# sampotter/butterfly

Measured on AMD Instinct MI355X. Metric: butterfly matvecs/sec (2D Helmholtz HODBF apply), higher is better.
Workload: dtype c128

## Files before the change

butterfly_amd/csrc/bfhip_stage_mfma.h:

```cpp
#ifndef BFHIP_STAGE_MFMA_H
#define BFHIP_STAGE_MFMA_H

#define BF_MF_TABCAP 1792u
#define BF_MF_TABPAD 24u
#define BF_MF_SPAN_BYTES (1u << 31)
#ifndef BF_MFMA_WAVES_PER_SIMD
#define BF_MFMA_WAVES_PER_SIMD 2
#endif
#ifndef BF_MF_XCD_RUN
#define BF_MF_XCD_RUN 32u
#endif
#ifndef BF_MF_WG_WAVES
#define BF_MF_WG_WAVES 1u
#endif
#ifndef BF_MFMA_MIN_RHS
#define BF_MFMA_MIN_RHS 2
#endif
#ifndef BF_MF_QUARTER
#define BF_MF_QUARTER 1
#endif

typedef double bf_d4 __attribute__((ext_vector_type(4)));
typedef int bf_i4 __attribute__((ext_vector_type(4)));
union BfFrag { bf_u4 u; double d[2]; };

__device__ __forceinline__ bf_i4 bfMakeRsrc(void const *base, uint32_t bytes) {
  uint64_t const b = (uint64_t)base;
  bf_i4 r;
  r.x = __builtin_amdgcn_readfirstlane((int)(uint32_t)b);
  r.y = __builtin_amdgcn_readfirstlane((int)((uint32_t)(b >> 32) & 0xffffu));
  r.z = __builtin_amdgcn_readfirstlane((int)bytes);
  r.w = 0x00020000;
  return r;
}
#ifndef BF_MF_A_POLICY
#define BF_MF_A_POLICY "nt"
#endif
template <int STREAM, int OFF> __device__ __forceinline__ void bfFragLoad(BfFrag &f, uint32_t voff, bf_i4 rsrc, uint32_t soff) {
  if (STREAM) asm volatile("buffer_load_dwordx4 %0, %1, %2, %3 offen offset:%4 " BF_MF_A_POLICY : "=v"(f.u) : "v"(voff), "s"(rsrc), "s"(soff), "n"(OFF));
  else asm volatile("buffer_load_dwordx4 %0, %1, %2, %3 offen offset:%4" : "=v"(f.u) : "v"(voff), "s"(rsrc), "s"(soff), "n"(OFF));
}
template <int N> __device__ __forceinline__ void bfFragWait(BfFrag &f) { asm volatile("s_waitcnt vmcnt(%1)" : "+v"(f.u) : "n"(N)); }
template <int N> __device__ __forceinline__ void bfFragWait(BfFrag &f, BfFrag &g) { asm volatile("s_waitcnt vmcnt(%2)" : "+v"(f.u), "+v"(g.u) : "n"(N)); }

struct BfMfSeg {
  bf_i4 ra, rx;
  uint32_t voffA;
  uint32_t cX;
  uint32_t stepA;
  uint32_t ksteps;
};

__device__ __forceinline__ void bfMfmaExact(bf_d4 &re, bf_d4 &im, BfFrag const &a, BfFrag const &x) {
  re = __builtin_amdgcn_mfma_f64_16x16x4f64(a.d[0], x.d[0], re, 0, 0, 0);
  re = __builtin_amdgcn_mfma_f64_16x16x4f64(a.d[1], x.d[1], re, 0, 0, 1);
  im = __builtin_amdgcn_mfma_f64_16x16x4f64(a.d[0], x.d[1], im, 0, 0, 0);
  im = __builtin_amdgcn_mfma_f64_16x16x4f64(a.d[1], x.d[0], im, 0, 0, 0);
}
template <int MS, int SET>
__device__ __forceinline__ void bfMfmaRequestA(BfFrag (&a)[2][2], BfMfSeg const &sg, uint32_t soffA) {
  bfFragLoad<1, 0>(a[SET][0], sg.voffA, sg.ra, soffA);
  if (MS > 1) bfFragLoad<1, 256>(a[SET][1], sg.voffA, sg.ra, soffA);
}
template <int T>
__device__ __forceinline__ void bfMfmaRequestX(BfFrag (&x)[4], BfMfSeg const &sg, uint32_t voffX) {
  bfFragLoad<0, 256 * T>(x[T], voffX, sg.rx, 0);
}
template <int NT, int MS, int SET, int T, bool GAUSS>
__device__ __forceinline__ void bfMfmaTile(bf_d4 (&acc)[3][2][4], BfFrag (&a)[2][2], BfFrag (&x)[4], double (&as)[2], BfMfSeg const &sg, uint32_t voffXnext) {
  if (T < NT) {
    constexpr int TT = T < NT ? T : 0;
    constexpr int pending = NT - 1 + MS;
    if (T == 0 && MS > 1) asm volatile("s_waitcnt vmcnt(%3)" : "+v"(a[SET][0].u), "+v"(a[SET][1].u), "+v"(x[0].u) : "n"(pending));
    else if (T == 0) asm volatile("s_waitcnt vmcnt(%2)" : "+v"(a[SET][0].u), "+v"(x[0].u) : "n"(pending));
    else asm volatile("s_waitcnt vmcnt(%1)" : "+v"(x[TT].u) : "n"(pending));
    if (GAUSS) {
      if (T == 0) {
        as[0] = a[SET][0].d[0] + a[SET][0].d[1];
        if (MS > 1) as[1] = a[SET][1].d[0] + a[SET][1].d[1];
      }
      double const xs = x[TT].d[0] + x[TT].d[1];
#pragma unroll
      for (int m = 0; m < MS; ++m) {
        acc[0][m][TT] = __builtin_amdgcn_mfma_f64_16x16x4f64(a[SET][m].d[0], x[TT].d[0], acc[0][m][TT], 0, 0, 0);
        acc[1][m][TT] = __builtin_amdgcn_mfma_f64_16x16x4f64(a[SET][m].d[1], x[TT].d[1], acc[1][m][TT], 0, 0, 0);
        acc[2][m][TT] = __builtin_amdgcn_mfma_f64_16x16x4f64(as[m], xs, acc[2][m][TT], 0, 0, 0);
      }
    } else {
#pragma unroll
      for (int m = 0; m < MS; ++m) bfMfmaExact(acc[0][m][TT], acc[1][m][TT], a[SET][m], x[TT]);
    }
    __builtin_amdgcn_sched_barrier(0);
    bfMfmaRequestX<TT>(x, sg, voffXnext);
    __builtin_amdgcn_sched_barrier(0);
  }
}
template <int NT, int MS, bool GAUSS = true>
__device__ __forceinline__ void bfMfmaSegment(bf_d4 (&acc)[3][2][4], BfMfSeg const &sg, uint32_t const *tab, uint32_t lk) {
  BfFrag a[2][2], x[4];
  double as[2];
  uint32_t ti = lk;
  uint32_t soffA = 0;
  {
    uint32_t const v0 = tab[ti] + sg.cX;
    bfMfmaRequestA<MS, 0>(a, sg, soffA);
    bfMfmaRequestX<0>(x, sg, v0);
    if (NT > 1) bfMfmaRequestX<1>(x, sg, v0);
    if (NT > 2) bfMfmaRequestX<2>(x, sg, v0);
    if (NT > 3) bfMfmaRequestX<3>(x, sg, v0);
  }
  uint32_t t1 = tab[ti + 4], t2 = tab[ti + 8];
  ti += 12;
  for (uint32_t ks = 0; ks < sg.ksteps; ks += 2) {
    uint32_t const v1 = t1 + sg.cX, v2 = t2 + sg.cX;
    t1 = tab[ti];
    t2 = tab[ti + 4];
    ti += 8;
    soffA += sg.stepA;
    __builtin_amdgcn_sched_barrier(0);
    bfMfmaRequestA<MS, 1>(a, sg, soffA);
    __builtin_amdgcn_sched_barrier(0);
    bfMfmaTile<NT, MS, 0, 0, GAUSS>(acc, a, x, as, sg, v1);
    bfMfmaTile<NT, MS, 0, 1, GAUSS>(acc, a, x, as, sg, v1);
    bfMfmaTile<NT, MS, 0, 2, GAUSS>(acc, a, x, as, sg, v1);
    bfMfmaTile<NT, MS, 0, 3, GAUSS>(acc, a, x, as, sg, v1);
    soffA += sg.stepA;
    bfMfmaRequestA<MS, 0>(a, sg, soffA);
    __builtin_amdgcn_sched_barrier(0);
    bfMfmaTile<NT, MS, 1, 0, GAUSS>(acc, a, x, as, sg, v2);
    bfMfmaTile<NT, MS, 1, 1, GAUSS>(acc, a, x, as, sg, v2);
    bfMfmaTile<NT, MS, 1, 2, GAUSS>(acc, a, x, as, sg, v2);
    bfMfmaTile<NT, MS, 1, 3, GAUSS>(acc, a, x, as, sg, v2);
  }
  asm volatile("s_waitcnt vmcnt(0)" : "+v"(a[0][0].u), "+v"(a[0][MS > 1 ? 1 : 0].u), "+v"(x[0].u), "+v"(x[NT > 1 ? 1 : 0].u), "+v"(x[NT > 2 ? 2 : 0].u), "+v"(x[NT > 3 ? 3 : 0].u));
}

template <int MS, int QT, int SET>
__device__ __forceinline__ void bfMfmaRequestAQ(BfFrag (&a)[2], BfFrag (&aq)[2][3], BfMfSeg const &sg, uint32_t voffAq, uint32_t soffA) {
  if (MS > 0) bfFragLoad<1, 0>(a[SET], sg.voffA, sg.ra, soffA);
  bfFragLoad<1, 256 * MS>(aq[SET][0], voffAq, sg.ra, soffA);
  if (QT > 1) bfFragLoad<1, 256 * MS + 64>(aq[SET][1], voffAq, sg.ra, soffA);
  if (QT > 2) bfFragLoad<1, 256 * MS + 128>(aq[SET][2], voffAq, sg.ra, soffA);
}
template <int MS, int QT, int SET, int T>
__device__ __forceinline__ void bfMfmaTileQ(bf_d4 (&acc)[3][4], double (&accq)[3][3][4], BfFrag (&a)[2], BfFrag (&aq)[2][3], BfFrag (&x)[4], double &as, double (&asq)[3],
                                            BfMfSeg const &sg, uint32_t voffXnext) {
  constexpr int pending = 4 - 1 + MS + QT;
  if (T == 0) {
    if (MS > 0 && QT == 1) asm volatile("s_waitcnt vmcnt(%3)" : "+v"(a[SET].u), "+v"(aq[SET][0].u), "+v"(x[0].u) : "n"(pending));
    else if (MS > 0 && QT == 2) asm volatile("s_waitcnt vmcnt(%4)" : "+v"(a[SET].u), "+v"(aq[SET][0].u), "+v"(aq[SET][1].u), "+v"(x[0].u) : "n"(pending));
    else if (MS > 0) asm volatile("s_waitcnt vmcnt(%5)" : "+v"(a[SET].u), "+v"(aq[SET][0].u), "+v"(aq[SET][1].u), "+v"(aq[SET][2].u), "+v"(x[0].u) : "n"(pending));
    else if (QT == 1) asm volatile("s_waitcnt vmcnt(%2)" : "+v"(aq[SET][0].u), "+v"(x[0].u) : "n"(pending));
    else if (QT == 2) asm volatile("s_waitcnt vmcnt(%3)" : "+v"(aq[SET][0].u), "+v"(aq[SET][1].u), "+v"(x[0].u) : "n"(pending));
    else asm volatile("s_waitcnt vmcnt(%4)" : "+v"(aq[SET][0].u), "+v"(aq[SET][1].u), "+v"(aq[SET][2].u), "+v"(x[0].u) : "n"(pending));
    if (MS > 0) as = a[SET].d[0] + a[SET].d[1];
#pragma unroll
    for (int q = 0; q < QT; ++q) asq[q] = aq[SET][q].d[0] + aq[SET][q].d[1];
  } else asm volatile("s_waitcnt vmcnt(%1)" : "+v"(x[T].u) : "n"(pending));
  double const xs = x[T].d[0] + x[T].d[1];
  if (MS > 0) {
    acc[0][T] = __builtin_amdgcn_mfma_f64_16x16x4f64(a[SET].d[0], x[T].d[0], acc[0][T], 0, 0, 0);
    acc[1][T] = __builtin_amdgcn_mfma_f64_16x16x4f64(a[SET].d[1], x[T].d[1], acc[1][T], 0, 0, 0);
    acc[2][T] = __builtin_amdgcn_mfma_f64_16x16x4f64(as, xs, acc[2][T], 0, 0, 0);
  }
#pragma unroll
  for (int q = 0; q < QT; ++q) {
    accq[0][q][T] = __builtin_amdgcn_mfma_f64_4x4x4f64(aq[SET][q].d[0], x[T].d[0], accq[0][q][T], 0, 0, 0);
    accq[1][q][T] = __builtin_amdgcn_mfma_f64_4x4x4f64(aq[SET][q].d[1], x[T].d[1], accq[1][q][T], 0, 0, 0);
    accq[2][q][T] = __builtin_amdgcn_mfma_f64_4x4x4f64(asq[q], xs, accq[2][q][T], 0, 0, 0);
  }
  __builtin_amdgcn_sched_barrier(0);
  bfMfmaRequestX<T>(x, sg, voffXnext);
  __builtin_amdgcn_sched_barrier(0);
}
template <int MS, int QT>
__device__ __forceinline__ void bfMfmaSegmentQ(bf_d4 (&acc)[3][4], double (&accq)[3][3][4], BfMfSeg const &sg, uint32_t voffAq, uint32_t const *tab, uint32_t lk) {
  BfFrag a[2], aq[2][3], x[4];
  double as = 0, asq[3];
  uint32_t ti = lk;
  uint32_t soffA = 0;
  {
    uint32_t const v0 = tab[ti] + sg.cX;
    bfMfmaRequestAQ<MS, QT, 0>(a, aq, sg, voffAq, soffA);
    bfMfmaRequestX<0>(x, sg, v0);
    bfMfmaRequestX<1>(x, sg, v0);
    bfMfmaRequestX<2>(x, sg, v0);
    bfMfmaRequestX<3>(x, sg, v0);
  }
  uint32_t t1 = tab[ti + 4], t2 = tab[ti + 8];
  ti += 12;
  for (uint32_t ks = 0; ks < sg.ksteps; ks += 2) {
    uint32_t const v1 = t1 + sg.cX, v2 = t2 + sg.cX;
    t1 = tab[ti];
    t2 = tab[ti + 4];
    ti += 8;
    soffA += sg.stepA;
    __builtin_amdgcn_sched_barrier(0);
    bfMfmaRequestAQ<MS, QT, 1>(a, aq, sg, voffAq, soffA);
    __builtin_amdgcn_sched_barrier(0);
    bfMfmaTileQ<MS, QT, 0, 0>(acc, accq, a, aq, x, as, asq, sg, v1);
    bfMfmaTileQ<MS, QT, 0, 1>(acc, accq, a, aq, x, as, asq, sg, v1);
    bfMfmaTileQ<MS, QT, 0, 2>(acc, accq, a, aq, x, as, asq, sg, v1);
    bfMfmaTileQ<MS, QT, 0, 3>(acc, accq, a, aq, x, as, asq, sg, v1);
    soffA += sg.stepA;
    bfMfmaRequestAQ<MS, QT, 0>(a, aq, sg, voffAq, soffA);
    __builtin_amdgcn_sched_barrier(0);
    bfMfmaTileQ<MS, QT, 1, 0>(acc, accq, a, aq, x, as, asq, sg, v2);
    bfMfmaTileQ<MS, QT, 1, 1>(acc, accq, a, aq, x, as, asq, sg, v2);
    bfMfmaTileQ<MS, QT, 1, 2>(acc, accq, a, aq, x, as, asq, sg, v2);
    bfMfmaTileQ<MS, QT, 1, 3>(acc, accq, a, aq, x, as, asq, sg, v2);
  }
  if (MS > 0) asm volatile("s_waitcnt vmcnt(0)" : "+v"(a[0].u) :: "memory");
  if (QT == 1) asm volatile("s_waitcnt vmcnt(0)" : "+v"(aq[0][0].u), "+v"(x[0].u), "+v"(x[1].u), "+v"(x[2].u), "+v"(x[3].u));
  else if (QT == 2) asm volatile("s_waitcnt vmcnt(0)" : "+v"(aq[0][0].u), "+v"(aq[0][1].u), "+v"(x[0].u), "+v"(x[1].u), "+v"(x[2].u), "+v"(x[3].u));
  else asm volatile("s_waitcnt vmcnt(0)" : "+v"(aq[0][0].u), "+v"(aq[0][1].u), "+v"(aq[0][2].u), "+v"(x[0].u), "+v"(x[1].u), "+v"(x[2].u), "+v"(x[3].u));
}
template <int MS, int QT>
__device__ __forceinline__ void bfMfmaStoreQ(StageParams const &p, BfDevItem const &it, uint32_t mr, uint32_t s0, uint32_t q0, double (&accq)[3][3][4], bool hasIdentity, int lane) {
  uint32_t const nrhs = p.nrhs, np = it.numPieces;
  double2 *out = (it.mrFlags & BF_ITEM_OUT_Y) ? (double2 *)p.y : (double2 *)p.temp;
  uint32_t const qmax = nrhs - 1 - q0;
  uint32_t lane2 = (uint32_t)lane;
  asm volatile("" : "+v"(lane2));
  uint32_t const li2 = lane2 & 15u, lk2 = lane2 >> 4;
#pragma unroll
  for (int q = 0; q < QT; ++q)
#pragma unroll
    for (int t = 0; t < 4; ++t) {
      uint32_t const row = s0 + 16u * MS + 4u * q + lk2;
      if (row < mr && 16u * t + li2 <= qmax) {
        double re = accq[0][q][t] - accq[1][q][t];
        double im = accq[2][q][t] - accq[0][q][t] - accq[1][q][t];
        if (hasIdentity) {
          for (uint32_t k = 0; k < np; ++k) {
            BfDevPiece const pc = p.pieces[it.pieceBegin + k];
            if (!(pc.flags & BF_PIECE_IDENTITY)) continue;
            double2 const *xin = (pc.flags & BF_PIECE_IN_X) ? (double2 const *)p.x : (double2 const *)p.temp;
            double2 xv = xin[((uint64_t)pc.inOff + row) * nrhs + q0 + 16 * t + li2];
            re += xv.x; im += xv.y;
          }
        }
        out[((uint64_t)it.outOff + row) * nrhs + q0 + 16 * t + li2] = make_double2(re, im);
      }
    }
}

template <int NT, int MS, bool GAUSS>
__device__ __forceinline__ void bfMfmaStore(StageParams const &p, BfDevItem const &it, uint32_t mr, uint32_t s0, uint32_t q0, bf_d4 (&acc)[3][2][4], bool hasIdentity, int lane) {
  uint32_t const nrhs = p.nrhs, np = it.numPieces;
  double2 *out = (it.mrFlags & BF_ITEM_OUT_Y) ? (double2 *)p.y : (double2 *)p.temp;
  uint32_t const qmax = nrhs - 1 - q0;
  uint32_t lane2 = (uint32_t)lane;
  asm volatile("" : "+v"(lane2));
  uint32_t const li2 = lane2 & 15u, lk2 = lane2 >> 4;
#pragma unroll
  for (int m = 0; m < MS; ++m)
#pragma unroll
    for (int t = 0; t < NT; ++t)
#pragma unroll
      for (int v = 0; v < 4; ++v) {
        uint32_t const row = s0 + 16u * m + 4 * v + lk2;
        if (row < mr && 16u * t + li2 <= qmax) {
          double re = GAUSS ? acc[0][m][t][v] - acc[1][m][t][v] : acc[0][m][t][v];
          double im = GAUSS ? acc[2][m][t][v] - acc[0][m][t][v] - acc[1][m][t][v] : acc[1][m][t][v];
          if (hasIdentity) {
            for (uint32_t k = 0; k < np; ++k) {
              BfDevPiece const pc = p.pieces[it.pieceBegin + k];
              if (!(pc.flags & BF_PIECE_IDENTITY)) continue;
              double2 const *xin = (pc.flags & BF_PIECE_IN_X) ? (double2 const *)p.x : (double2 const *)p.temp;
              double2 xv = xin[((uint64_t)pc.inOff + row) * nrhs + q0 + 16 * t + li2];
              re += xv.x; im += xv.y;
            }
          }
          out[((uint64_t)it.outOff + row) * nrhs + q0 + 16 * t + li2] = make_double2(re, im);
        }
      }
}

template <int NT, int MS, bool GAUSS, int QT = 0>
__device__ __forceinline__ void bfMfmaPass(StageParams const &p, BfDevItem const &it, uint32_t mr, uint32_t s0, uint32_t q0, uint32_t *tab, int lane) {
  static_assert(QT == 0 || (NT == 4 && MS <= 1 && GAUSS), "quarter slabs: the 4-tile Gauss register loop");
  asm volatile("s_waitcnt vmcnt(0)" ::: "memory");
  uint32_t const nrhs = p.nrhs;
  uint32_t const li = lane & 15, lk = lane >> 4;
  bf_d4 acc[3][2][4];
  bf_d4 accs[3][4];
  double accq[3][3][4];
#pragma unroll
  for (int g = 0; g < 3; ++g)
#pragma unroll
    for (int m = 0; m < MS; ++m)
#pragma unroll
      for (int t = 0; t < NT; ++t) acc[g][m][t] = (bf_d4){0, 0, 0, 0};
  if (QT > 0) {
#pragma unroll
    for (int g = 0; g < 3; ++g)
#pragma unroll
      for (int t = 0; t < 4; ++t) {
        accs[g][t] = (bf_d4){0, 0, 0, 0};
#pragma unroll
        for (int q = 0; q < 3; ++q) accq[g][q][t] = 0.0;
      }
  }
  bool hasIdentity = false;
  uint32_t const np = it.numPieces;
  uint32_t const spanRows = BF_MF_SPAN_BYTES / (nrhs * 16u);
  uint32_t pi = 0;
  while (pi < np) {
    uint32_t cols = 0, minRow = 0, maxRow = 0, inX = 0;
    uint64_t aOff = 0, expect = 0;
    bool started = false;
    BfPieceWin win;
    uint32_t wbase = 0xffffff00u;
    while (pi < np) {
      if (pi - wbase >= 64u) {
        wbase = pi;
        win = bfPieceWinLoad(p.pieces + it.pieceBegin + wbase, np - wbase < 64u ? np - wbase : 64u, lane);
      }
      BfDevPiece const pc = bfPieceWinGet(win, pi - wbase);
      if (pc.flags & BF_PIECE_IDENTITY) { hasIdentity = true; ++pi; continue; }
      uint32_t const px = pc.flags & BF_PIECE_IN_X, last = pc.inOff + pc.ncols - 1;
      uint32_t lo = pc.inOff, hi = last;
      if (started) {
        if (pc.dataOff != expect || px != inX || cols + pc.ncols > BF_MF_TABCAP) break;
        lo = minRow < lo ? minRow : lo;
        hi = maxRow > hi ? maxRow : hi;
        if (hi - lo >= spanRows) break;
      } else {
        started = true;
        aOff = pc.dataOff;
        inX = px;
      }
      minRow = lo;
      maxRow = hi;
      for (uint32_t j = (uint32_t)lane; j < pc.ncols; j += 64u) tab[cols + j] = pc.inOff + j;
      cols += pc.ncols;
      expect = pc.dataOff + (uint64_t)mr * pc.ncols;
      ++pi;
    }
    if (!cols) break;
    if ((uint32_t)lane < BF_MF_TABPAD) tab[cols + lane] = minRow;
    waveSync();
    for (uint32_t j = (uint32_t)lane; j < cols + BF_MF_TABPAD; j += 64u) tab[j] = (tab[j] - minRow) * (nrhs * 16u);
    waveSync();
    BfMfSeg sg;
    sg.stepA = 4u * mr * 16u;
    sg.ksteps = (cols + 3u) / 4u;
    sg.ra = bfMakeRsrc((double2 const *)p.arena + aOff, mr * cols * 16u);
    char const *xin = inX ? (char const *)p.x : (char const *)p.temp;
    sg.rx = bfMakeRsrc(xin + ((uint64_t)minRow * nrhs + q0) * 16u, ((maxRow - minRow) * nrhs + (nrhs - q0)) * 16u);
    sg.voffA = (lk * mr + s0 + li) * 16u;
    sg.cX = li * 16u;
    if constexpr (QT > 0) bfMfmaSegmentQ<MS, QT>(accs, accq, sg, (lk * mr + s0 + (li & 3u)) * 16u, tab, lk);
    else bfMfmaSegment<NT, MS, GAUSS>(acc, sg, tab, lk);
    waveSync();
  }
  if constexpr (QT > 0) {
    bfMfmaStoreQ<MS, QT>(p, it, mr, s0, q0, accq, hasIdentity, lane);
    if (MS > 0) {
#pragma unroll
      for (int g = 0; g < 3; ++g)
#pragma unroll
        for (int t = 0; t < 4; ++t) acc[g][0][t] = accs[g][t];
    }
  }
  bfMfmaStore<NT, MS, GAUSS>(p, it, mr, s0, q0, acc, hasIdentity, lane);
}

template <int MS, int MAXNT, bool GAUSS>
__device__ __forceinline__ void bfMfmaDispatch(uint32_t nt, StageParams const &p, BfDevItem const &it, uint32_t mr, uint32_t s0, uint32_t q0, uint32_t *tab, int lane) {
  if (MAXNT >= 4 && nt == 4) bfMfmaPass<4, MS, GAUSS>(p, it, mr, s0, q0, tab, lane);
  else if (MAXNT >= 3 && nt == 3) bfMfmaPass<3, MS, GAUSS>(p, it, mr, s0, q0, tab, lane);
  else if (MAXNT >= 2 && nt == 2) bfMfmaPass<2, MS, GAUSS>(p, it, mr, s0, q0, tab, lane);
  else bfMfmaPass<1, MS, GAUSS>(p, it, mr, s0, q0, tab, lane);
}

template <int MAXNT, int WAVES, bool GAUSS = true>
__device__ __forceinline__ void bfStageBodyC128Mfma(StageParams const &p, uint32_t (*tabs)[BF_MF_TABCAP + BF_MF_TABPAD]) {
  int const lane = threadIdx.x & 63;
  uint32_t const wave = __builtin_amdgcn_readfirstlane(threadIdx.x >> 6);
  uint32_t *tab = tabs[wave];
  uint32_t wg = blockIdx.x;
  uint32_t const numWg = (p.numItems + BF_MF_WG_WAVES - 1u) / BF_MF_WG_WAVES;
  if (BF_MF_XCD_RUN > 1) {
    uint32_t const blk = 8u * BF_MF_XCD_RUN;
    if (wg < numWg / blk * blk) { uint32_t const r = wg % blk; wg = wg - r + (r % 8u) * BF_MF_XCD_RUN + r / 8u; }
  }
  uint32_t const item = wg * BF_MF_WG_WAVES + wave;
  if (item >= p.numItems) return;
  BfDevItem const it = p.items[item];
  uint32_t const mr = it.mrFlags & 0xffffu;
  uint32_t const nrhs = p.nrhs;
  for (uint32_t q0 = 0; q0 < nrhs; q0 += 64) {
    uint32_t const nt = (nrhs - q0 >= 64) ? 4u : (nrhs - q0 + 15u) / 16u;
    uint32_t s0 = 0;
    while (s0 < mr) {
      uint32_t const left = mr - s0;
      if (BF_MF_QUARTER && MAXNT == 4 && GAUSS && nt == 4 && left < 32 && (left & 15u) && (left & 15u) <= 12u) {
        if constexpr (MAXNT == 4 && GAUSS) {
          uint32_t const qt = ((left & 15u) + 3u) / 4u;
          if (left > 16) {
            if (qt == 1) bfMfmaPass<4, 1, true, 1>(p, it, mr, s0, q0, tab, lane);
            else if (qt == 2) bfMfmaPass<4, 1, true, 2>(p, it, mr, s0, q0, tab, lane);
            else bfMfmaPass<4, 1, true, 3>(p, it, mr, s0, q0, tab, lane);
          } else {
            if (qt == 1) bfMfmaPass<4, 0, true, 1>(p, it, mr, s0, q0, tab, lane);
            else if (qt == 2) bfMfmaPass<4, 0, true, 2>(p, it, mr, s0, q0, tab, lane);
            else bfMfmaPass<4, 0, true, 3>(p, it, mr, s0, q0, tab, lane);
          }
        }
        s0 = mr;
      }
      else if (left > 16) { bfMfmaDispatch<2, MAXNT, GAUSS>(nt, p, it, mr, s0, q0, tab, lane); s0 += 32; }
      else { bfMfmaDispatch<1, MAXNT, GAUSS>(nt, p, it, mr, s0, q0, tab, lane); s0 += 16; }
    }
  }
}

__global__ __launch_bounds__(64 * BF_MF_WG_WAVES) __attribute__((amdgpu_waves_per_eu(BF_MFMA_WAVES_PER_SIMD, BF_MFMA_WAVES_PER_SIMD))) void bfStageKernelC128Mfma(StageParams p) {
  __shared__ uint32_t tabs[BF_MF_WG_WAVES][BF_MF_TABCAP + BF_MF_TABPAD];
  bfStageBodyC128Mfma<4, BF_MFMA_WAVES_PER_SIMD>(p, tabs);
}
__global__ __launch_bounds__(64 * BF_MF_WG_WAVES) __attribute__((amdgpu_waves_per_eu(3, 3))) void bfStageKernelC128Mfma2(StageParams p) {
  __shared__ uint32_t tabs[BF_MF_WG_WAVES][BF_MF_TABCAP + BF_MF_TABPAD];
  bfStageBodyC128Mfma<2, 3>(p, tabs);
}
__global__ __launch_bounds__(64 * BF_MF_WG_WAVES) __attribute__((amdgpu_waves_per_eu(5, 5))) void bfStageKernelC128Mfma1(StageParams p) {
  __shared__ uint32_t tabs[BF_MF_WG_WAVES][BF_MF_TABCAP + BF_MF_TABPAD];
  bfStageBodyC128Mfma<1, 5>(p, tabs);
}
__global__ __launch_bounds__(64 * BF_MF_WG_WAVES) __attribute__((amdgpu_waves_per_eu(BF_MFMA_WAVES_PER_SIMD, BF_MFMA_WAVES_PER_SIMD))) void bfStageKernelC128MfmaExact(StageParams p) {
  __shared__ uint32_t tabs[BF_MF_WG_WAVES][BF_MF_TABCAP + BF_MF_TABPAD];
  bfStageBodyC128Mfma<4, BF_MFMA_WAVES_PER_SIMD, false>(p, tabs);
}
__global__ __launch_bounds__(64 * BF_MF_WG_WAVES) __attribute__((amdgpu_waves_per_eu(3, 3))) void bfStageKernelC128Mfma2Exact(StageParams p) {
  __shared__ uint32_t tabs[BF_MF_WG_WAVES][BF_MF_TABCAP + BF_MF_TABPAD];
  bfStageBodyC128Mfma<2, 3, false>(p, tabs);
}
__global__ __launch_bounds__(64 * BF_MF_WG_WAVES) __attribute__((amdgpu_waves_per_eu(5, 5))) void bfStageKernelC128Mfma1Exact(StageParams p) {
  __shared__ uint32_t tabs[BF_MF_WG_WAVES][BF_MF_TABCAP + BF_MF_TABPAD];
  bfStageBodyC128Mfma<1, 5, false>(p, tabs);
}
#endif
```

Measured before the change: 95.53.

## Add deep-ring MFMA pipelines for narrow RHS quarter tiles and exact path

Adds a templated multi-stage load ring (RING buffered A/X fragments with vmcnt-based waits) for the 1-tile MFMA kernels. When the remaining RHS columns are 8 or fewer, it uses 4x4x4 f64 MFMAs on 4-column quarter tiles with a Gauss 3-multiply scheme, so it no longer computes full 16-wide tiles for padded columns. The non-Gauss exact path also gets a deeper ring. The goal is to hide memory latency and cut wasted MFMA work on narrow right-hand sides, at the cost of more registers and more template instantiations.

Result: no change. 95.54 (median of 3 runs) (+0.0%).

```diff
diff --git a/butterfly_amd/csrc/bfhip_stage_mfma.h b/butterfly_amd/csrc/bfhip_stage_mfma.h
--- a/butterfly_amd/csrc/bfhip_stage_mfma.h
+++ b/butterfly_amd/csrc/bfhip_stage_mfma.h
@@ -18,6 +18,24 @@
 #endif
 #ifndef BF_MF_QUARTER
 #define BF_MF_QUARTER 1
+#endif
+#ifndef BF_MF_FEW_QUARTER
+#define BF_MF_FEW_QUARTER 1
+#endif
+#ifndef BF_MF_RING_Q4
+#define BF_MF_RING_Q4 5
+#endif
+#ifndef BF_MF_RING_Q8
+#define BF_MF_RING_Q8 2
+#endif
+#ifndef BF_MF_RING_Q4_ONE
+#define BF_MF_RING_Q4_ONE ((BF_MF_RING_Q4 + 3) & ~1)
+#endif
+#ifndef BF_MF_RING_Q8_ONE
+#define BF_MF_RING_Q8_ONE ((BF_MF_RING_Q8 + 2) & ~1)
+#endif
+#ifndef BF_MF_RING_EXACT
+#define BF_MF_RING_EXACT 3
 #endif
 
 typedef double bf_d4 __attribute__((ext_vector_type(4)));
@@ -133,6 +151,112 @@
     bfMfmaTile<NT, MS, 1, 3, GAUSS>(acc, a, x, as, sg, v2);
   }
   asm volatile("s_waitcnt vmcnt(0)" : "+v"(a[0][0].u), "+v"(a[0][MS > 1 ? 1 : 0].u), "+v"(x[0].u), "+v"(x[NT > 1 ? 1 : 0].u), "+v"(x[NT > 2 ? 2 : 0].u), "+v"(x[NT > 3 ? 3 : 0].u));
+}
+
+template <int MS, int NX, int RING, int SET>
+__device__ __forceinline__ void bfRingRequest(BfFrag (&a)[RING][2], BfFrag (&x)[RING][2], BfMfSeg const &sg, uint32_t soffA, uint32_t voffX) {
+  bfFragLoad<1, 0>(a[SET][0], sg.voffA, sg.ra, soffA);
+  if (MS > 1) bfFragLoad<1, 256>(a[SET][1], sg.voffA, sg.ra, soffA);
+  bfFragLoad<0, 0>(x[SET][0], voffX, sg.rx, 0);
+  if (NX > 1) bfFragLoad<0, 64>(x[SET][1], voffX, sg.rx, 0);
+}
+template <int MS, int NX, int RING, int SET, int PENDING>
+__device__ __forceinline__ void bfRingWait(BfFrag (&a)[RING][2], BfFrag (&x)[RING][2]) {
+  if (MS > 1 && NX > 1) asm volatile("s_waitcnt vmcnt(%4)" : "+v"(a[SET][0].u), "+v"(a[SET][1].u), "+v"(x[SET][0].u), "+v"(x[SET][1].u) : "n"(PENDING));
+  else if (MS > 1) asm volatile("s_waitcnt vmcnt(%3)" : "+v"(a[SET][0].u), "+v"(a[SET][1].u), "+v"(x[SET][0].u) : "n"(PENDING));
+  else if (NX > 1) asm volatile("s_waitcnt vmcnt(%3)" : "+v"(a[SET][0].u), "+v"(x[SET][0].u), "+v"(x[SET][1].u) : "n"(PENDING));
+  else asm volatile("s_waitcnt vmcnt(%2)" : "+v"(a[SET][0].u), "+v"(x[SET][0].u) : "n"(PENDING));
+}
+template <int MS, int NX>
+__device__ __forceinline__ void bfRingMul(double (&acc)[3][2][2], BfFrag const (&a)[2], BfFrag const (&x)[2]) {
+  double as[2], xs[2];
+#pragma unroll
+  for (int m = 0; m < MS; ++m) as[m] = a[m].d[0] + a[m].d[1];
+#pragma unroll
+  for (int g = 0; g < NX; ++g) xs[g] = x[g].d[0] + x[g].d[1];
+#pragma unroll
+  for (int g = 0; g < NX; ++g)
+#pragma unroll
+    for (int m = 0; m < MS; ++m) {
+      acc[0][m][g] = __builtin_amdgcn_mfma_f64_4x4x4f64(a[m].d[0], x[g].d[0], acc[0][m][g], 0, 0, 0);
+      acc[1][m][g] = __builtin_amdgcn_mfma_f64_4x4x4f64(a[m].d[1], x[g].d[1], acc[1][m][g], 0, 0, 0);
+      acc[2][m][g] = __builtin_amdgcn_mfma_f64_4x4x4f64(as[m], xs[g], acc[2][m][g], 0, 0, 0);
+    }
+}
+template <int MS, int NX>
+__device__ __forceinline__ void bfRingMul(bf_d4 (&acc)[3][2][4], BfFrag const (&a)[2], BfFrag const (&x)[2]) {
+  static_assert(NX == 1, "the exact ring loop: one X tile");
+#pragma unroll
+  for (int m = 0; m < MS; ++m) bfMfmaExact(acc[0][m][0], acc[1][m][0], a[m], x[0]);
+}
+template <int MS, int NX, int RING, int I, class ACC>
+__device__ __forceinline__ void bfRingPrologue(BfFrag (&a)[RING][2], BfFrag (&x)[RING][2], BfMfSeg const &sg, uint32_t const *tab, uint32_t lk, uint32_t &soffA) {
+  if constexpr (I < RING) {
+    uint32_t const kq = (uint32_t)I < sg.ksteps ? (uint32_t)I : sg.ksteps;
+    bfRingRequest<MS, NX, RING, I>(a, x, sg, soffA, tab[lk + 4u * kq] + sg.cX);
+    soffA += sg.stepA;
+    bfRingPrologue<MS, NX, RING, I + 1, ACC>(a, x, sg, tab, lk, soffA);
+  }
+}
+template <int MS, int NX, int RING, int I, class ACC>
+__device__ __forceinline__ void bfRingSteps(ACC &acc, BfFrag (&a)[RING][2], BfFrag (&x)[RING][2], BfMfSeg const &sg, uint32_t const *tab, uint32_t lk, uint32_t ks, uint32_t &soffA) {
+  if constexpr (I < RING) {
+    uint32_t const kn = ks + (uint32_t)(I + RING);
+    uint32_t const tn = tab[lk + 4u * (kn < sg.ksteps ? kn : sg.ksteps)];
+    __builtin_amdgcn_sched_barrier(0);
+    bfRingWait<MS, NX, RING, I, (RING - 1) * (MS + NX)>(a, x);
+    bfRingMul<MS, NX>(acc, a[I], x[I]);
+    __builtin_amdgcn_sched_barrier(0);
+    bfRingRequest<MS, NX, RING, I>(a, x, sg, soffA, tn + sg.cX);
+    __builtin_amdgcn_sched_barrier(0);
+    soffA += sg.stepA;
+    bfRingSteps<MS, NX, RING, I + 1, ACC>(acc, a, x, sg, tab, lk, ks, soffA);
+  }
+}
+template <int MS, int NX, int RING, int I>
+__device__ __forceinline__ void bfRingDrain(BfFrag (&a)[RING][2], BfFrag (&x)[RING][2]) {
+  if constexpr (I < RING) {
+    bfRingWait<MS, NX, RING, I, 0>(a, x);
+    bfRingDrain<MS, NX, RING, I + 1>(a, x);
+  }
+}
+template <int MS, int NX, int RING, class ACC>
+__device__ __forceinline__ void bfMfmaSegmentRing(ACC &acc, BfMfSeg const &sg, uint32_t const *tab, uint32_t lk) {
+  static_assert(RING >= 2 && (RING - 1) * (MS + NX) < 64, "vmcnt has six bits");
+  BfFrag a[RING][2], x[RING][2];
+  uint32_t soffA = 0;
+  bfRingPrologue<MS, NX, RING, 0, ACC>(a, x, sg, tab, lk, soffA);
+  for (uint32_t ks = 0; ks < sg.ksteps; ks += RING) bfRingSteps<MS, NX, RING, 0, ACC>(acc, a, x, sg, tab, lk, ks, soffA);
+  bfRingDrain<MS, NX, RING, 0>(a, x);
+}
+template <int MS, int NX>
+__device__ __forceinline__ void bfMfmaStoreF(StageParams const &p, BfDevItem const &it, uint32_t mr, uint32_t s0, uint32_t q0, double (&acc)[3][2][2], bool hasIdentity, int lane) {
+  uint32_t const nrhs = p.nrhs, np = it.numPieces;
+  double2 *out = (it.mrFlags & BF_ITEM_OUT_Y) ? (double2 *)p.y : (double2 *)p.temp;
+  uint32_t const qmax = nrhs - 1 - q0;
+  uint32_t lane2 = (uint32_t)lane;
+  asm volatile("" : "+v"(lane2));
+  uint32_t const lj = lane2 & 3u, lrow = 4u * ((lane2 >> 2) & 3u) + (lane2 >> 4);
+#pragma unroll
+  for (int m = 0; m < MS; ++m)
+#pragma unroll
+    for (int g = 0; g < NX; ++g) {
+      uint32_t const row = s0 + 16u * m + lrow, col = 4u * g + lj;
+      if (row < mr && col <= qmax) {
+        double re = acc[0][m][g] - acc[1][m][g];
+        double im = acc[2][m][g] - acc[0][m][g] - acc[1][m][g];
+        if (hasIdentity) {
+          for (uint32_t k = 0; k < np; ++k) {
+            BfDevPiece const pc = p.pieces[it.pieceBegin + k];
+            if (!(pc.flags & BF_PIECE_IDENTITY)) continue;
+            double2 const *xin = (pc.flags & BF_PIECE_IN_X) ? (double2 const *)p.x : (double2 const *)p.temp;
+            double2 xv = xin[((uint64_t)pc.inOff + row) * nrhs + q0 + col];
+            re += xv.x; im += xv.y;
+          }
+        }
+        out[((uint64_t)it.outOff + row) * nrhs + q0 + col] = make_double2(re, im);
+      }
+    }
 }
 
 template <int MS, int QT, int SET>
@@ -277,21 +401,31 @@
       }
 }
 
-template <int NT, int MS, bool GAUSS, int QT = 0>
+template <int NT, int MS, bool GAUSS, int QT = 0, int NQ = 0, int RING = 2>
 __device__ __forceinline__ void bfMfmaPass(StageParams const &p, BfDevItem const &it, uint32_t mr, uint32_t s0, uint32_t q0, uint32_t *tab, int lane) {
   static_assert(QT == 0 || (NT == 4 && MS <= 1 && GAUSS), "quarter slabs: the 4-tile Gauss register loop");
+  static_assert(NQ == 0 || (NT == 1 && QT == 0 && GAUSS), "quarter-tile passes: the 1-tile Gauss kernel");
+  static_assert(RING == 2 || (NT == 1 && QT == 0 && MS >= 1), "the ring loop: the 1-tile kernels");
   asm volatile("s_waitcnt vmcnt(0)" ::: "memory");
   uint32_t const nrhs = p.nrhs;
   uint32_t const li = lane & 15, lk = lane >> 4;
   bf_d4 acc[3][2][4];
   bf_d4 accs[3][4];
   double accq[3][3][4];
-#pragma unroll
-  for (int g = 0; g < 3; ++g)
-#pragma unroll
-    for (int m = 0; m < MS; ++m)
-#pragma unroll
-      for (int t = 0; t < NT; ++t) acc[g][m][t] = (bf_d4){0, 0, 0, 0};
+  double accf[3][2][2];
+  if constexpr (NQ > 0) {
+#pragma unroll
+    for (int g = 0; g < 3; ++g)
+#pragma unroll
+      for (int m = 0; m < 2; ++m) accf[g][m][0] = accf[g][m][1] = 0.0;
+  } else {
+#pragma unroll
+    for (int g = 0; g < 3; ++g)
+#pragma unroll
+      for (int m = 0; m < MS; ++m)
+#pragma unroll
+        for (int t = 0; t < NT; ++t) acc[g][m][t] = (bf_d4){0, 0, 0, 0};
+  }
   if (QT > 0) {
 #pragma unroll
     for (int g = 0; g < 3; ++g)
@@ -350,8 +484,10 @@
     char const *xin = inX ? (char const *)p.x : (char const *)p.temp;
     sg.rx = bfMakeRsrc(xin + ((uint64_t)minRow * nrhs + q0) * 16u, ((maxRow - minRow) * nrhs + (nrhs - q0)) * 16u);
     sg.voffA = (lk * mr + s0 + li) * 16u;
-    sg.cX = li * 16u;
-    if constexpr (QT > 0) bfMfmaSegmentQ<MS, QT>(accs, accq, sg, (lk * mr + s0 + (li & 3u)) * 16u, tab, lk);
+    sg.cX = NQ > 0 ? (li & 3u) * 16u : li * 16u;
+    if constexpr (NQ > 0) bfMfmaSegmentRing<MS, NQ, RING>(accf, sg, tab, lk);
+    else if constexpr (RING > 2) bfMfmaSegmentRing<MS, 1, RING>(acc, sg, tab, lk);
+    else if constexpr (QT > 0) bfMfmaSegmentQ<MS, QT>(accs, accq, sg, (lk * mr + s0 + (li & 3u)) * 16u, tab, lk);
     else bfMfmaSegment<NT, MS, GAUSS>(acc, sg, tab, lk);
     waveSync();
   }
@@ -364,7 +500,8 @@
         for (int t = 0; t < 4; ++t) acc[g][0][t] = accs[g][t];
     }
   }
-  bfMfmaStore<NT, MS, GAUSS>(p, it, mr, s0, q0, acc, hasIdentity, lane);
+  if constexpr (NQ > 0) bfMfmaStoreF<MS, NQ>(p, it, mr, s0, q0, accf, hasIdentity, lane);
+  else bfMfmaStore<NT, MS, GAUSS>(p, it, mr, s0, q0, acc, hasIdentity, lane);
 }
 
 template <int MS, int MAXNT, bool GAUSS>
@@ -372,6 +509,7 @@
   if (MAXNT >= 4 && nt == 4) bfMfmaPass<4, MS, GAUSS>(p, it, mr, s0, q0, tab, lane);
   else if (MAXNT >= 3 && nt == 3) bfMfmaPass<3, MS, GAUSS>(p, it, mr, s0, q0, tab, lane);
   else if (MAXNT >= 2 && nt == 2) bfMfmaPass<2, MS, GAUSS>(p, it, mr, s0, q0, tab, lane);
+  else if (MAXNT == 1 && !GAUSS && BF_MF_RING_EXACT > 2) bfMfmaPass<1, MS, GAUSS, 0, 0, (MAXNT == 1 && !GAUSS && BF_MF_RING_EXACT > 2) ? BF_MF_RING_EXACT : 2>(p, it, mr, s0, q0, tab, lane);
   else bfMfmaPass<1, MS, GAUSS>(p, it, mr, s0, q0, tab, lane);
 }
 
@@ -411,6 +549,20 @@
         }
         s0 = mr;
       }
+      else if (BF_MF_FEW_QUARTER && MAXNT == 1 && GAUSS && nrhs - q0 <= 8) {
+        if constexpr (BF_MF_FEW_QUARTER && MAXNT == 1 && GAUSS) {
+          constexpr int R41 = BF_MF_RING_Q4_ONE, R81 = BF_MF_RING_Q8_ONE;
+          static_assert(R41 % 2 == 0, "one slab, one group: 3 MFMAs per k-step -- an even ring keeps the loop's MFMA count even");
+          if (nrhs - q0 <= 4) {
+            if (left > 16) bfMfmaPass<1, 2, true, 0, 1, BF_MF_RING_Q4>(p, it, mr, s0, q0, tab, lane);
+            else bfMfmaPass<1, 1, true, 0, 1, R41>(p, it, mr, s0, q0, tab, lane);
+          } else {
+            if (left > 16) bfMfmaPass<1, 2, true, 0, 2, BF_MF_RING_Q8>(p, it, mr, s0, q0, tab, lane);
+            else bfMfmaPass<1, 1, true, 0, 2, R81>(p, it, mr, s0, q0, tab, lane);
+          }
+        }
+        s0 += left > 16 ? 32 : 16;
+      }
       else if (left > 16) { bfMfmaDispatch<2, MAXNT, GAUSS>(nt, p, it, mr, s0, q0, tab, lane); s0 += 32; }
       else { bfMfmaDispatch<1, MAXNT, GAUSS>(nt, p, it, mr, s0, q0, tab, lane); s0 += 16; }
     }
```

## Use three-slot prefetch pipeline with exact products for one-tile MFMA kernel

Applied to the files above, without the earlier changes.

The single-tile MFMA stage kernel now runs a new segment loop that keeps three A/X fragment slots in flight, two loads ahead, instead of the two-slot parent loop. It also switches that kernel from the Gauss three-product complex multiply to the exact four-product form. The deeper prefetch is meant to hide global load latency for narrow-RHS stages, at the cost of more live registers at an occupancy of five waves per SIMD. The four-product path does more MFMA work but drops the Gauss combination arithmetic. A macro restores the old loop.

Result: no change. 95.06 before, 95.63 after, median of 3 (+0.6%).

```diff
diff --git a/butterfly_amd/csrc/bfhip_stage_mfma.h b/butterfly_amd/csrc/bfhip_stage_mfma.h
--- a/butterfly_amd/csrc/bfhip_stage_mfma.h
+++ b/butterfly_amd/csrc/bfhip_stage_mfma.h
@@ -15,6 +15,9 @@
 #endif
 #ifndef BF_MFMA_MIN_RHS
 #define BF_MFMA_MIN_RHS 2
+#endif
+#ifndef BF_MF1_PARENT_LOOP
+#define BF_MF1_PARENT_LOOP 0
 #endif
 #ifndef BF_MF_QUARTER
 #define BF_MF_QUARTER 1
@@ -133,6 +136,51 @@
     bfMfmaTile<NT, MS, 1, 3, GAUSS>(acc, a, x, as, sg, v2);
   }
   asm volatile("s_waitcnt vmcnt(0)" : "+v"(a[0][0].u), "+v"(a[0][MS > 1 ? 1 : 0].u), "+v"(x[0].u), "+v"(x[NT > 1 ? 1 : 0].u), "+v"(x[NT > 2 ? 2 : 0].u), "+v"(x[NT > 3 ? 3 : 0].u));
+}
+
+template <int MS, int SLOT>
+__device__ __forceinline__ void bfMfmaRequest3(BfFrag (&a)[3][2], BfFrag (&x)[3], BfMfSeg const &sg, uint32_t soffA, uint32_t voffX) {
+  bfFragLoad<1, 0>(a[SLOT][0], sg.voffA, sg.ra, soffA);
+  if (MS > 1) bfFragLoad<1, 256>(a[SLOT][1], sg.voffA, sg.ra, soffA);
+  bfFragLoad<0, 0>(x[SLOT], voffX, sg.rx, 0);
+}
+template <int MS, int SLOT>
+__device__ __forceinline__ void bfMfmaStep3(bf_d4 (&acc)[3][2][4], BfFrag (&a)[3][2], BfFrag (&x)[3], BfMfSeg const &sg, uint32_t soffA, uint32_t voffX) {
+  constexpr int pending = 2 * (MS + 1);
+  __builtin_amdgcn_sched_barrier(0);
+  bfMfmaRequest3<MS, (SLOT + 2) % 3>(a, x, sg, soffA, voffX);
+  __builtin_amdgcn_sched_barrier(0);
+  if (MS > 1) asm volatile("s_waitcnt vmcnt(%3)" : "+v"(a[SLOT][0].u), "+v"(a[SLOT][1].u), "+v"(x[SLOT].u) : "n"(pending));
+  else asm volatile("s_waitcnt vmcnt(%2)" : "+v"(a[SLOT][0].u), "+v"(x[SLOT].u) : "n"(pending));
+#pragma unroll
+  for (int m = 0; m < MS; ++m) bfMfmaExact(acc[0][m][0], acc[1][m][0], a[SLOT][m], x[SLOT]);
+}
+template <int MS>
+__device__ __forceinline__ void bfMfmaSegment3(bf_d4 (&acc)[3][2][4], BfMfSeg const &sg, uint32_t const *tab, uint32_t lk) {
+  BfFrag a[3][2], x[3];
+  uint32_t ti = lk;
+  uint32_t soffA = sg.stepA;
+  bfMfmaRequest3<MS, 0>(a, x, sg, 0, tab[ti] + sg.cX);
+  bfMfmaRequest3<MS, 1>(a, x, sg, soffA, tab[ti + 4] + sg.cX);
+  uint32_t t = tab[ti + 8];
+  ti += 12;
+  for (uint32_t ks = 0; ks < sg.ksteps; ks += 3) {
+    uint32_t const v2 = t + sg.cX;
+    t = tab[ti];
+    soffA += sg.stepA;
+    bfMfmaStep3<MS, 0>(acc, a, x, sg, soffA, v2);
+    uint32_t const v3 = t + sg.cX;
+    t = tab[ti + 4];
+    soffA += sg.stepA;
+    bfMfmaStep3<MS, 1>(acc, a, x, sg, soffA, v3);
+    uint32_t const v4 = t + sg.cX;
+    t = tab[ti + 8];
+    ti += 12;
+    soffA += sg.stepA;
+    bfMfmaStep3<MS, 2>(acc, a, x, sg, soffA, v4);
+  }
+  if (MS > 1) asm volatile("s_waitcnt vmcnt(0)" : "+v"(a[0][0].u), "+v"(a[0][1].u), "+v"(a[1][0].u), "+v"(a[1][1].u), "+v"(a[2][0].u), "+v"(a[2][1].u), "+v"(x[0].u), "+v"(x[1].u), "+v"(x[2].u));
+  else asm volatile("s_waitcnt vmcnt(0)" : "+v"(a[0][0].u), "+v"(a[1][0].u), "+v"(a[2][0].u), "+v"(x[0].u), "+v"(x[1].u), "+v"(x[2].u));
 }
 
 template <int MS, int QT, int SET>
@@ -277,9 +325,10 @@
       }
 }
 
-template <int NT, int MS, bool GAUSS, int QT = 0>
+template <int NT, int MS, bool GAUSS, int QT = 0, int SLOTS = 2>
 __device__ __forceinline__ void bfMfmaPass(StageParams const &p, BfDevItem const &it, uint32_t mr, uint32_t s0, uint32_t q0, uint32_t *tab, int lane) {
   static_assert(QT == 0 || (NT == 4 && MS <= 1 && GAUSS), "quarter slabs: the 4-tile Gauss register loop");
+  static_assert(SLOTS == 2 || (SLOTS == 3 && NT == 1 && !GAUSS && QT == 0), "three slots: the one-tile four-product loop");
   asm volatile("s_waitcnt vmcnt(0)" ::: "memory");
   uint32_t const nrhs = p.nrhs;
   uint32_t const li = lane & 15, lk = lane >> 4;
@@ -352,6 +401,7 @@
     sg.voffA = (lk * mr + s0 + li) * 16u;
     sg.cX = li * 16u;
     if constexpr (QT > 0) bfMfmaSegmentQ<MS, QT>(accs, accq, sg, (lk * mr + s0 + (li & 3u)) * 16u, tab, lk);
+    else if constexpr (SLOTS == 3) bfMfmaSegment3<MS>(acc, sg, tab, lk);
     else bfMfmaSegment<NT, MS, GAUSS>(acc, sg, tab, lk);
     waveSync();
   }
@@ -372,7 +422,7 @@
   if (MAXNT >= 4 && nt == 4) bfMfmaPass<4, MS, GAUSS>(p, it, mr, s0, q0, tab, lane);
   else if (MAXNT >= 3 && nt == 3) bfMfmaPass<3, MS, GAUSS>(p, it, mr, s0, q0, tab, lane);
   else if (MAXNT >= 2 && nt == 2) bfMfmaPass<2, MS, GAUSS>(p, it, mr, s0, q0, tab, lane);
-  else bfMfmaPass<1, MS, GAUSS>(p, it, mr, s0, q0, tab, lane);
+  else bfMfmaPass<1, MS, GAUSS, 0, (MAXNT == 1 && !GAUSS && !BF_MF1_PARENT_LOOP) ? 3 : 2>(p, it, mr, s0, q0, tab, lane);
 }
 
 template <int MAXNT, int WAVES, bool GAUSS = true>
@@ -427,7 +477,7 @@
 }
 __global__ __launch_bounds__(64 * BF_MF_WG_WAVES) __attribute__((amdgpu_waves_per_eu(5, 5))) void bfStageKernelC128Mfma1(StageParams p) {
   __shared__ uint32_t tabs[BF_MF_WG_WAVES][BF_MF_TABCAP + BF_MF_TABPAD];
-  bfStageBodyC128Mfma<1, 5>(p, tabs);
+  bfStageBodyC128Mfma<1, 5, BF_MF1_PARENT_LOOP != 0>(p, tabs);
 }
 __global__ __launch_bounds__(64 * BF_MF_WG_WAVES) __attribute__((amdgpu_waves_per_eu(BF_MFMA_WAVES_PER_SIMD, BF_MFMA_WAVES_PER_SIMD))) void bfStageKernelC128MfmaExact(StageParams p) {
   __shared__ uint32_t tabs[BF_MF_WG_WAVES][BF_MF_TABCAP + BF_MF_TABPAD];
```
